# Crocodoctopus/zkstark

Hardware: AMD Instinct MI355X
Metric: field-elements/s through LDE+Merkle+FRI (full STARK-101 prover) (higher is better)
Workload: dtype u32 (mod 3*2^30+1) + SHA-256

## Files before the change

zkstark_amd/csrc/kernels.hip:

```cpp
#include "kernels.hpp"

#include <cstdlib>

#include "blake2s.hpp"
#include "field.hpp"
#include "fieldhash_f64.hpp"
#include "sha256_quad.hpp"
#include "sha256.hpp"

namespace zk {

__device__ __forceinline__ uint32_t pow_lookup(const PowTable& t, uint32_t e) {
    return mont_mul(t.hi[e >> t.lo_bits], t.lo[e & ((1u << t.lo_bits) - 1u)]);
}

constexpr uint32_t R2_MONT = R2;

__device__ uint32_t mont_inv(uint32_t a) {
    uint32_t r = R1, b = a;
    uint32_t e = P - 2;
#pragma unroll 1
    for (int i = 0; i < 32; ++i) {
        if (e & 1) r = mont_mul(r, b);
        b = mont_mul(b, b);
// ... 908 lines not shown
    }
    __syncthreads();
    for (uint32_t q = tid; q < np; q += nt) out[(size_t)q * a.out_stride] = high[q];
}
hipError_t launch_fri_final_poly_batch(const FinalPolyArgs& a, hipStream_t s, Profiler* prof) {
    if (a.log_m < 1 || a.log_m > kFinalPolyMaxLog || a.log_m > a.L || a.polys < 1 || !a.in || !a.out) return hipErrorInvalidValue;
    const uint32_t M = 1u << a.log_m;
    if (a.bound < 1 || a.bound > M || a.in_stride != M || a.out_stride != (size_t)a.bound + 1) return hipErrorInvalidValue;
    uint32_t per = (1u << kFinalPolyMaxLog) >> a.log_m;
    if (per > kFinalPolyBatchMaxPer) per = kFinalPolyBatchMaxPer;
    ScopedKernelTimer tm(prof, K_FOLD, 4.0 * (double)a.polys * (double)(M + a.bound + 1), s);
    const uint32_t most = (a.polys < per ? a.polys : per) << (a.log_m - 1);
    const uint32_t threads = most >= kFinalPolyThreads ? kFinalPolyThreads : ((most + 63u) & ~63u);
    hipLaunchKernelGGL(fri_final_poly_batch_kernel, dim3((a.polys + per - 1) / per), dim3(threads), 0, s, a, per);
    return hipGetLastError();
}


__constant__ FieldHashConsts g_fh_consts;
__constant__ FieldHashConsts64 g_fh_consts64;

template <int HASH> struct Hasher;
template <> struct Hasher<0> {
    static __device__ __forceinline__ Digest leaf(uint32_t v) { return sha256_leaf(v); }
    static __device__ __forceinline__ Digest inner(const Digest& l, const Digest& r) { return sha256_inner(l, r); }
};
template <> struct Hasher<1> {
    static __device__ __forceinline__ Digest leaf(uint32_t v) { return fieldhash_leaf64(v, g_fh_consts64); }
    static __device__ __forceinline__ Digest inner(const Digest& l, const Digest& r) { return fieldhash_inner64(l, r, g_fh_consts64); }
};
template <> struct Hasher<2> {
    static __device__ __forceinline__ Digest leaf(uint32_t v) { return blake2s_leaf(v); }
    static __device__ __forceinline__ Digest inner(const Digest& l, const Digest& r) { return blake2s_inner(l, r); }
};

struct PlainSrc {
    const uint32_t* vals;
    using Raw = uint32_t;
    __device__ __forceinline__ Raw fetch(size_t pos) const { return vals[pos]; }
    __device__ __forceinline__ uint32_t finish(const Raw& r, size_t) const { return r; }
    __device__ __forceinline__ uint32_t load(size_t pos) const { return vals[pos]; }
};
struct FoldSrc {
    FoldArgs a;
    using Raw = FoldRaw;
    __device__ __forceinline__ void prepare() { if (a.dyn) a.c_mont = *a.dyn; }
    __device__ __forceinline__ Raw fetch(size_t pos) const { return fold_fetch(a, pos); }
    __device__ __forceinline__ uint32_t finish(const Raw& r, size_t pos) const { uint32_t v = fold_finish(a, r); a.out[pos] = v; return v; }
    __device__ __forceinline__ uint32_t load(size_t pos) const { return finish(fetch(pos), pos); }
};
struct ComposeSrc {
    ComposeArgs a;
    using Raw = size_t;
    __device__ __forceinline__ Raw fetch(size_t pos) const { return pos; }
    __device__ __forceinline__ uint32_t finish(const Raw& r, size_t) const { return load(r); }
    __device__ __forceinline__ uint32_t load(size_t pos) const { uint32_t v = compose_at(a, pos); a.cp[pos] = v; return v; }
};

struct ComposeBlockSrc {
    ComposeBlockArgs b;
    using Raw = size_t;
    __device__ __forceinline__ uint32_t f_at(size_t t) const {
        const uint32_t gmask = (1u << b.lg) - 1u;
        if (t >> b.log_m) {
            const size_t v = t - ((size_t)1 << b.log_m);
            return b.halo[(v & gmask) * b.halo_stride + (v >> b.lg)];
        }
        const uint32_t log_cl = b.lg + b.log_cnt;
        const size_t piece = ((t >> log_cl) << b.lg) | (t & gmask);
        return b.a.f[(piece << b.log_cnt) | ((t & (((size_t)1 << log_cl) - 1)) >> b.lg)];
    }
    __device__ __forceinline__ Raw fetch(size_t pos) const { return pos; }
    __device__ __forceinline__ uint32_t finish(const Raw& r, size_t) const { return load(r); }
    __device__ __forceinline__ uint32_t load(size_t pos) const {
        const ComposeArgs& a = b.a;
        const size_t B = (size_t)1 << a.log_b;
        const uint32_t f0 = f_at(pos), f1 = f_at(pos + B), f2 = f_at(pos + 2 * B);
        const uint32_t x = mont_mul(pow_lookup(a.htab, b.e0 + (uint32_t)pos), a.w_mont);
        return compose_eval<false>(a, f0, f1, f2, a.inv_xm1[pos], a.inv_xm1[pos + 2 * B], x, a.zz[pos & (B - 1)], a.first, a.last, a.alpha0_mont,
                                   a.alpha1g2_mont, 0u);
    }
};

struct ComposeBatchSrc {
    ComposeArgs a;
    const BatchChal* chal;
    using Raw = size_t;
    __device__ __forceinline__ Raw fetch(size_t pos) const { return pos; }
    __device__ __forceinline__ uint32_t finish(const Raw& r, size_t) const { return load(r); }
    __device__ __forceinline__ uint32_t load(size_t pos) const {
        const size_t b = pos >> a.logN, i = pos & (((size_t)1 << a.logN) - 1);
        const BatchChal c = chal[b];
        uint32_t v = compose_core<true>(a, a.f + (b << a.logN), c.first, c.last, c.alpha0_mont, c.alpha1g2_mont, c.alpha2_mont, i);
        a.cp[pos] = v;
        return v;
    }
};
struct FoldBatchSrc {
    FoldArgs a;
    const BatchChal* chal;
    using Raw = size_t;
    __device__ __forceinline__ Raw fetch(size_t pos) const { return pos; }
    __device__ __forceinline__ uint32_t finish(const Raw& r, size_t) const { return load(r); }
    __device__ __forceinline__ uint32_t load(size_t pos) const {
        const uint32_t lh = a.log_m - 1;
        const size_t half = (size_t)1 << lh, b = pos >> lh, i = pos & (half - 1);
        const uint32_t* in = a.in + (b << a.log_m);
        uint32_t u = in[i], v = in[i + half];
        uint32_t xinv = pow_lookup(a.hinv, (uint32_t)(i << a.round));
        uint32_t s = mont_mul(add(u, v), a.inv2_mont);
        uint32_t d = mont_mul(mont_mul(sub(u, v), xinv), chal[b].c_mont);
        uint32_t r = add(s, d);
        a.out[pos] = r;
        return r;
    }
};

struct InterleaveSrc {
    const uint32_t* recv;
    uint32_t log_parts, log_cnt;
    using Raw = uint32_t;
    __device__ __forceinline__ uint32_t load(size_t pos) const {
        return recv[((pos & (((size_t)1 << log_parts) - 1)) << log_cnt) | (pos >> log_parts)];
    }
    __device__ __forceinline__ Raw fetch(size_t pos) const { return load(pos); }
    __device__ __forceinline__ uint32_t finish(const Raw& r, size_t) const { return r; }
};

template <class S> __device__ __forceinline__ auto src_prepare(S& s, int) -> decltype(s.prepare(), void()) { s.prepare(); }
template <class S> __device__ __forceinline__ void src_prepare(S&, long) {}

constexpr int kMerkleThreads = 256;
constexpr uint32_t kMerkleMaxK = 4;

__device__ __forceinline__ void store_digest(uint32_t* nodes, size_t node, const Digest& d) {
    uint4* q = reinterpret_cast<uint4*>(nodes + node * 8);
    q[0] = make_uint4(d.w[0], d.w[1], d.w[2], d.w[3]);
    q[1] = make_uint4(d.w[4], d.w[5], d.w[6], d.w[7]);
}
__device__ __forceinline__ Digest load_digest(const uint32_t* nodes, size_t node) {
    const uint4* q = reinterpret_cast<const uint4*>(nodes + node * 8);
    uint4 lo = q[0], hi = q[1];
    Digest d;
    d.w[0] = lo.x; d.w[1] = lo.y; d.w[2] = lo.z; d.w[3] = lo.w;
    d.w[4] = hi.x; d.w[5] = hi.y; d.w[6] = hi.z; d.w[7] = hi.w;
    return d;
}

__device__ __forceinline__ Digest lds_digest(const uint4* p) {
    uint4 lo = p[0], hi = p[1];
    Digest d;
    d.w[0] = lo.x; d.w[1] = lo.y; d.w[2] = lo.z; d.w[3] = lo.w;
    d.w[4] = hi.x; d.w[5] = hi.y; d.w[6] = hi.z; d.w[7] = hi.w;
    return d;
}

template <class SRC, bool LEAF, int HASH>
__global__ __launch_bounds__(kMerkleThreads) void merkle_subtree_kernel(SRC src, uint32_t* nodes,
                                                                        uint32_t depth_in, uint32_t k, size_t off) {
    extern __shared__ __attribute__((aligned(16))) uint4 stage[];
    src_prepare(src, 0);
    const uint32_t lane = threadIdx.x & 63u, wave = threadIdx.x >> 6;
    const size_t gwave = (size_t)blockIdx.x * (kMerkleThreads / 64) + wave;
    const size_t base = (gwave << (6 + k)) + off;
    const size_t in_base = ((size_t)1 << depth_in) - 1;
    uint4* my = stage + (size_t)wave * (k + 1) * 128;
    uint4* scratch = my + (size_t)k * 128;
    typename SRC::Raw raw;
    Digest dnext;
    uint32_t val = 0;
    if (LEAF) val = src.load(base + lane - off);
    else dnext = load_digest(nodes, in_base + base + lane);
#pragma unroll 1
    for (uint32_t i = 0; i < (1u << k); ++i) {
        Digest d;
        const size_t pos = base + (size_t)i * 64 + lane;
        const bool more = i + 1 < (1u << k);
        if (LEAF) {
            if (more) raw = src.fetch(pos + 64 - off);
            d = Hasher<HASH>::leaf(val);
            store_digest(nodes, in_base + pos, d);
        } else {
            d = dnext;
            if (more) dnext = load_digest(nodes, in_base + pos + 64);
        }
        uint32_t idx = i, lvl = 0;
#pragma unroll 1
        while (lvl < k) {
            uint4* left = my + lvl * 128;
            uint4* grp = (idx & 1u) ? scratch : left;
            grp[2 * lane] = make_uint4(d.w[0], d.w[1], d.w[2], d.w[3]);
            grp[2 * lane + 1] = make_uint4(d.w[4], d.w[5], d.w[6], d.w[7]);
            if (!(idx & 1u)) break;
            __builtin_amdgcn_fence(__ATOMIC_RELEASE, "wavefront");
            __builtin_amdgcn_wave_barrier();
            const uint4* x = (lane < 32u ? left : scratch - 128) + 4 * lane;
            Digest l = lds_digest(x), r = lds_digest(x + 2);
            __builtin_amdgcn_wave_barrier();
            d = Hasher<HASH>::inner(l, r);
            idx >>= 1;
            ++lvl;
            store_digest(nodes, (((size_t)1 << (depth_in - lvl)) - 1) + (base >> lvl) + (size_t)idx * 64 + lane, d);
        }
        if (LEAF && more) val = src.finish(raw, pos + 64 - off);
    }
}

template <class SRC> struct B2sSrc { static constexpr bool ok = false; };
template <> struct B2sSrc<PlainSrc> { static constexpr bool ok = true; };
template <> struct B2sSrc<ComposeSrc> { static constexpr bool ok = true; };
template <> struct B2sSrc<FoldSrc> { static constexpr bool ok = true; };

template <class SRC, bool LEAF>
__global__ __launch_bounds__(kMerkleThreads) void b2s_subtree_kernel(SRC src, uint32_t* nodes, uint32_t depth_in, uint32_t k, size_t off) {
    extern __shared__ __attribute__((aligned(16))) uint4 stage[];
    src_prepare(src, 0);
    const uint32_t lane = threadIdx.x & 63u, wave = threadIdx.x >> 6;
    const size_t gwave = (size_t)blockIdx.x * (kMerkleThreads / 64) + wave;
    const size_t base = (gwave << (6 + k)) + off;
    const size_t in_base = ((size_t)1 << depth_in) - 1;
    uint4* my = stage + (size_t)wave * (k + 1) * 128;
    uint4* scratch = my + (size_t)k * 128;
    typename SRC::Raw raw;
    Digest dnext;
    uint32_t val = 0;
    if (LEAF) val = src.load(base + lane - off);
    else dnext = load_digest(nodes, in_base + base + lane);
#pragma unroll 1
    for (uint32_t i = 0; i < (1u << k); ++i) {
        Digest d;
        const size_t pos = base + (size_t)i * 64 + lane;
        const bool more = i + 1 < (1u << k);
        if (LEAF) {
            if (more) raw = src.fetch(pos + 64 - off);
            d = blake2s_leaf(val);
            store_digest(nodes, in_base + pos, d);
        } else {
            d = dnext;
            if (more) dnext = load_digest(nodes, in_base + pos + 64);
        }
        uint32_t idx = i, lvl = 0;
#pragma unroll 1
        while (lvl < k) {
            uint4* left = my + lvl * 128;
            uint4* grp = (idx & 1u) ? scratch : left;
            grp[2 * lane] = make_uint4(d.w[0], d.w[1], d.w[2], d.w[3]);
            grp[2 * lane + 1] = make_uint4(d.w[4], d.w[5], d.w[6], d.w[7]);
            if (!(idx & 1u)) break;
            __builtin_amdgcn_fence(__ATOMIC_RELEASE, "wavefront");
            __builtin_amdgcn_wave_barrier();
            const uint4* x = (lane < 32u ? left : scratch - 128) + 4 * lane;
            const Digest l = lds_digest(x), r = lds_digest(x + 2);
            __builtin_amdgcn_wave_barrier();
            d = blake2s_inner(l, r);
            idx >>= 1;
            ++lvl;
            store_digest(nodes, (((size_t)1 << (depth_in - lvl)) - 1) + (base >> lvl) + (size_t)idx * 64 + lane, d);
        }
        if (LEAF && more) val = src.finish(raw, pos + 64 - off);
    }
}

constexpr int kWgThreads = 256;
#ifndef ZK_FIELD_ROW_MAX_NODES
#define ZK_FIELD_ROW_MAX_NODES 16
#endif
constexpr uint32_t kFieldRowMaxNodes = ZK_FIELD_ROW_MAX_NODES;
static_assert(kFieldRowMaxNodes >= 16 && kFieldRowMaxNodes <= 64, "the row form takes at most four passes of 16 nodes");
#ifndef ZK_FIELD_QUAD_MAX_NODES
#define ZK_FIELD_QUAD_MAX_NODES 64
#endif
constexpr uint32_t kFieldQuadMaxNodes = ZK_FIELD_QUAD_MAX_NODES;
static_assert(kFieldQuadMaxNodes <= 128, "the quad form takes at most two passes of 64 nodes");
#ifndef ZK_FIELD_ROW_LEAF_MAX
#define ZK_FIELD_ROW_LEAF_MAX 32
#endif
constexpr uint32_t kFieldRowLeafMax = ZK_FIELD_ROW_LEAF_MAX;
static_assert(kFieldRowLeafMax <= 64, "the row form takes at most four passes of 16 leaves");
constexpr uint32_t kWgMaxLog = 10;

__device__ __forceinline__ void lds_store(uint4* p, const Digest& d) {
    p[0] = make_uint4(d.w[0], d.w[1], d.w[2], d.w[3]);
    p[1] = make_uint4(d.w[4], d.w[5], d.w[6], d.w[7]);
}

#ifndef ZK_WG_RELAXED_PUBLISH
#define ZK_WG_RELAXED_PUBLISH 1
#endif
constexpr bool kWgRelaxedPublish = ZK_WG_RELAXED_PUBLISH != 0;
__device__ __forceinline__ void publish_node(uint32_t* nodes, size_t node, const uint4* lvl0, uint32_t tid) {
    if (tid < 8) __hip_atomic_store(nodes + node * 8 + tid, reinterpret_cast<const uint32_t*>(lvl0)[tid], __ATOMIC_RELAXED, __HIP_MEMORY_SCOPE_AGENT);
    asm volatile("s_waitcnt vmcnt(0)" ::: "memory");
}
__device__ __forceinline__ Digest load_digest_agent(const uint32_t* nodes, size_t node) {
    const unsigned long long* q = reinterpret_cast<const unsigned long long*>(nodes + node * 8);
    Digest d;
#pragma unroll
    for (int i = 0; i < 4; ++i) {
        const unsigned long long v = __hip_atomic_load(q + i, __ATOMIC_RELAXED, __HIP_MEMORY_SCOPE_AGENT);
        d.w[2 * i] = (uint32_t)v; d.w[2 * i + 1] = (uint32_t)(v >> 32);
    }
    return d;
}

#ifdef ZK_WG_TRACE
constexpr uint32_t kWgTraceSlots = 48, kWgTraceLaunches = 8192;
__device__ unsigned long long g_wg_trace[kWgTraceLaunches][kWgTraceSlots];
__device__ unsigned int g_wg_trace_n, g_wg_trace_cur;
#define WG_STAMP(slot) do { if (threadIdx.x == 0 && wg_rec < kWgTraceLaunches && (slot) < kWgTraceSlots) g_wg_trace[wg_rec][(slot)] = __builtin_amdgcn_s_memrealtime(); } while (0)
#else
#define WG_STAMP(slot) do { } while (0)
#endif

template <class SRC, bool LEAF, int HASH>
__global__ __launch_bounds__(kWgThreads) void merkle_wg_kernel(SRC src, uint32_t* nodes, uint32_t depth_in, uint32_t j,
                                                               MailArgs mail, size_t off, uint32_t j2, uint32_t lds_log) {
    extern __shared__ __attribute__((aligned(16))) uint4 lvl[];
    src_prepare(src, 0);
    uint32_t* xch = reinterpret_cast<uint32_t*>(lvl + ((size_t)2 << lds_log));
    const uint32_t tid = threadIdx.x;
    uint32_t cnt = 1u << j;
    size_t first = ((size_t)blockIdx.x << j) + off;
    uint32_t d_in = depth_in, lv = j;
    const size_t in_base = ((size_t)1 << depth_in) - 1;
    QuadLane ql;
    if (HASH == 0) ql = quad_lane(tid);
#ifdef ZK_WG_TRACE
    uint32_t wg_rec = 0xffffffffu;
    if (blockIdx.x == 0 && tid == 0) {
        wg_rec = atomicAdd(&g_wg_trace_n, 1u);
        __hip_atomic_store(&g_wg_trace_cur, wg_rec, __ATOMIC_RELAXED, __HIP_MEMORY_SCOPE_AGENT);
        if (wg_rec < kWgTraceLaunches) {
            for (uint32_t i = 0; i < kWgTraceSlots; ++i) g_wg_trace[wg_rec][i] = 0;
            g_wg_trace[wg_rec][0] = (unsigned long long)depth_in | ((unsigned long long)j << 8) | ((unsigned long long)j2 << 16) | ((unsigned long long)(LEAF ? 1 : 0) << 24) |
                                    ((unsigned long long)HASH << 25) | ((unsigned long long)(mail.mailbox ? mail.top + 1 : 0) << 26) | ((unsigned long long)gridDim.x << 32);
        }
    }
    WG_STAMP(1);
#endif
    constexpr uint32_t kPer = (1u << kWgMaxLog) / kWgThreads;
    if (LEAF && HASH == 1 && cnt <= kFieldRowLeafMax) {
        const uint32_t g = tid & 15u, grp = tid >> 4;
#pragma unroll 1
        for (uint32_t b = 0; b * 16 < cnt; ++b) {
            const uint32_t i = b * 16 + grp;
            const uint32_t ii = i < cnt ? i : 0u;
            const uint32_t v = src.finish(src.fetch(first + ii - off), first + ii - off);
            const uint32_t word = g == 0 ? v : g == 15 ? 1u : 0u;
            const uint32_t res = fieldhash_inner_row16_f64(word, g, g_fh_consts64);
            if (i < cnt && g < 8) {
                nodes[(in_base + first + i) * 8 + g] = res;
                reinterpret_cast<uint32_t*>(&lvl[2 * i])[g] = res;
            }
        }
    } else if (LEAF) {
        typename SRC::Raw raw[kPer] = {};
#pragma unroll
        for (uint32_t u = 0; u < kPer; ++u)
            if (tid + u * kWgThreads < cnt) raw[u] = src.fetch(first + tid + u * kWgThreads - off);
#pragma unroll 1
        for (uint32_t i = tid; i < cnt; i += kWgThreads) {
            const Digest d = Hasher<HASH>::leaf(src.finish(raw[0], first + i - off));
            store_digest(nodes, in_base + first + i, d);
            lds_store(&lvl[2 * i], d);
#pragma unroll
            for (uint32_t u = 0; u + 1 < kPer; ++u) raw[u] = raw[u + 1];
        }
    } else {
        Digest dd[kPer];
#pragma unroll
        for (uint32_t u = 0; u < kPer; ++u)
            if (tid + u * kWgThreads < cnt) dd[u] = load_digest(nodes, in_base + first + tid + u * kWgThreads);
#pragma unroll
        for (uint32_t u = 0; u < kPer; ++u)
            if (tid + u * kWgThreads < cnt) lds_store(&lvl[2 * (tid + u * kWgThreads)], dd[u]);
    }
    if (LEAF && mail.dump_src) __threadfence();
    __syncthreads();
    WG_STAMP(2);
#pragma unroll 1
  for (uint32_t phase = 0;; ++phase) {
#pragma unroll 1
    for (uint32_t t = 1; t <= lv; ++t) {
        const uint32_t w = cnt >> t;
        const size_t out_base = (((size_t)1 << (d_in - t)) - 1) + (first >> t);
        WG_STAMP((phase ? 24u : 2u) + t - 1u);
        if (HASH == 0 && w <= 64) {
            const uint32_t lane = tid & 63u, wave = tid >> 6;
            const uint32_t node = wave * 16 + (lane >> 4) * 4 + (lane & 3u), role = (lane >> 2) & 3u;
            const bool busy = wave * 16 < w;
            uint32_t o[4];
            if (busy) sha256_inner_quad(reinterpret_cast<const uint32_t*>(&lvl[4 * (node < w ? node : 0u)]), ql, o);
            __syncthreads();
            if (busy && node < w && role < 2) {
                const uint4 v = make_uint4(o[0], o[1], o[2], o[3]);
                lvl[2 * node + (role ^ 1u)] = v;
                reinterpret_cast<uint4*>(nodes + (out_base + node) * 8)[role ^ 1u] = v;
            }
            __syncthreads();
            continue;
        }
        if (HASH == 0 && w <= 128) {
            const bool is_main = tid < 128;
            const uint32_t node = tid & 127u;
            const bool active = node < w;
            uint32_t wv[16];
            uint32_t st[8];
            if (active) {
                Digest l = lds_digest(&lvl[4 * node]), r = lds_digest(&lvl[4 * node + 2]);
#pragma unroll
                for (int i = 0; i < 8; ++i) { wv[i] = l.w[i]; wv[8 + i] = r.w[i]; st[i] = SHA_IV[i]; }
            }
            uint32_t* xb0 = xch;
            uint32_t* xb1 = xch + 16 * 128;
            if (active) {
                if (is_main) sha256_rounds16<0>(st, wv);
                else { sha256_schedule16(wv);
#pragma unroll
                       for (int i = 0; i < 16; ++i) xb0[i * 128 + node] = wv[i]; }
            }
            __syncthreads();
            if (active) {
                if (is_main) {
#pragma unroll
                    for (int i = 0; i < 16; ++i) wv[i] = xb0[i * 128 + node];
                    sha256_rounds16<16>(st, wv);
                } else { sha256_schedule16(wv);
#pragma unroll
                         for (int i = 0; i < 16; ++i) xb1[i * 128 + node] = wv[i]; }
            }
            __syncthreads();
            if (active) {
                if (is_main) {
#pragma unroll
                    for (int i = 0; i < 16; ++i) wv[i] = xb1[i * 128 + node];
                    sha256_rounds16<32>(st, wv);
                } else { sha256_schedule16(wv);
#pragma unroll
                         for (int i = 0; i < 16; ++i) xb0[i * 128 + node] = wv[i]; }
            }
            __syncthreads();
            Digest d0;
            if (active && is_main) {
#pragma unroll
                for (int i = 0; i < 16; ++i) wv[i] = xb0[i * 128 + node];
                sha256_rounds16<48>(st, wv);
#pragma unroll
                for (int i = 0; i < 8; ++i) d0.w[i] = st[i] + SHA_IV[i];
                uint32_t pad[16] = {0x80000000u, 0, 0, 0, 0, 0, 0, 0, 0, 0, 0, 0, 0, 0, 0, 512u};
                sha256_compress(d0.w, pad);
            }
            __syncthreads();
            if (active && is_main) { lds_store(&lvl[2 * node], d0); store_digest(nodes, out_base + node, d0); }
            __syncthreads();
            continue;
        }
        if (HASH == 1 && w > kFieldRowMaxNodes && w <= kFieldQuadMaxNodes) {
            const uint32_t q = tid & 3u, grp = tid >> 2;
            uint32_t res[2][4];
#pragma unroll
            for (uint32_t b = 0; b < 2; ++b) {
                if (b * 64 >= w) break;
                const uint32_t node = b * 64 + grp;
                const uint4 v = lvl[4 * (node < w ? node : 0u) + q];
                const uint32_t in[4] = {v.x, v.y, v.z, v.w};
                fieldhash_inner_quad_f64(in, q, res[b], g_fh_consts64);
            }
            __syncthreads();
#pragma unroll
            for (uint32_t b = 0; b < 2; ++b) {
                if (b * 64 >= w) break;
                const uint32_t node = b * 64 + grp;
                if (node < w && q < 2) {
                    const uint4 o = make_uint4(res[b][0], res[b][1], res[b][2], res[b][3]);
                    lvl[2 * node + q] = o;
                    reinterpret_cast<uint4*>(nodes + (out_base + node) * 8)[q] = o;
                }
            }
            __syncthreads();
            continue;
        }
        if (HASH == 1 && w <= kFieldRowMaxNodes) {
            const uint32_t g = tid & 15u, grp = tid >> 4;
            uint32_t res[4];
#pragma unroll
            for (uint32_t b = 0; b < 4; ++b) {
                if (b * 16 >= w) break;
                const uint32_t node = b * 16 + grp;
                const uint32_t* words = reinterpret_cast<const uint32_t*>(&lvl[4 * (node < w ? node : 0u)]);
                res[b] = fieldhash_inner_row16_f64(words[g], g, g_fh_consts64);
            }
            __syncthreads();
#pragma unroll
            for (uint32_t b = 0; b < 4; ++b) {
                if (b * 16 >= w) break;
                const uint32_t node = b * 16 + grp;
                if (node < w && g < 8) {
                    reinterpret_cast<uint32_t*>(&lvl[2 * node])[g] = res[b];
                    nodes[(out_base + node) * 8 + g] = res[b];
                }
            }
            __syncthreads();
            continue;
        }
        Digest d0, d1;
        const bool a0 = tid < w, a1 = tid + kWgThreads < w;
        if (a0) d0 = Hasher<HASH>::inner(lds_digest(&lvl[4 * tid]), lds_digest(&lvl[4 * tid + 2]));
        if (a1) d1 = Hasher<HASH>::inner(lds_digest(&lvl[4 * (tid + kWgThreads)]), lds_digest(&lvl[4 * (tid + kWgThreads) + 2]));
        __syncthreads();
        if (a0) { lds_store(&lvl[2 * tid], d0); store_digest(nodes, out_base + tid, d0); }
        if (a1) { lds_store(&lvl[2 * (tid + kWgThreads)], d1); store_digest(nodes, out_base + tid + kWgThreads, d1); }
        __syncthreads();
    }
    WG_STAMP((phase ? 24u : 2u) + lv);
    if (phase == 1 || j2 == 0) break;
    __shared__ uint32_t go_on;
    if (gridDim.x > 1) {
        if (kWgRelaxedPublish) {
            publish_node(nodes, (((size_t)1 << (depth_in - j)) - 1) + blockIdx.x, lvl, tid);
        } else {
            asm volatile("s_waitcnt vmcnt(0)" ::: "memory");
            __syncthreads();
        }
    }
    if (tid == 0) {
        uint32_t last = 1;
        if (gridDim.x > 1) {
            last = (kWgRelaxedPublish ? __hip_atomic_fetch_add(mail.counter + 1, 1u, __ATOMIC_RELAXED, __HIP_MEMORY_SCOPE_AGENT)
                                      : __hip_atomic_fetch_add(mail.counter + 1, 1u, __ATOMIC_ACQ_REL, __HIP_MEMORY_SCOPE_AGENT)) == gridDim.x - 1;
            if (last) __hip_atomic_store(mail.counter + 1, 0u, __ATOMIC_RELAXED, __HIP_MEMORY_SCOPE_AGENT);
        }
        go_on = last;
    }
    __syncthreads();
    if (!go_on) return;
    if (kWgRelaxedPublish && LEAF && mail.dump_src) __builtin_amdgcn_fence(__ATOMIC_ACQUIRE, "agent");
#ifdef ZK_WG_TRACE
    if (tid == 0) wg_rec = __hip_atomic_load(&g_wg_trace_cur, __ATOMIC_RELAXED, __HIP_MEMORY_SCOPE_AGENT);
    WG_STAMP(15);
#endif
    d_in = depth_in - j; lv = j2; cnt = gridDim.x; first = 0;
    {
        const size_t base2 = ((size_t)1 << d_in) - 1;
        Digest dd[kPer];
#pragma unroll
        for (uint32_t u = 0; u < kPer; ++u)
            if (tid + u * kWgThreads < cnt)
                dd[u] = (kWgRelaxedPublish && gridDim.x > 1) ? load_digest_agent(nodes, base2 + tid + u * kWgThreads) : load_digest(nodes, base2 + tid + u * kWgThreads);
#pragma unroll
        for (uint32_t u = 0; u < kPer; ++u)
            if (tid + u * kWgThreads < cnt) lds_store(&lvl[2 * (tid + u * kWgThreads)], dd[u]);
    }
    __syncthreads();
    WG_STAMP(16);
  }
    if (mail.mailbox && depth_in - j - j2 == mail.top && off == 0) {
        __shared__ uint32_t is_last;
        const bool relaxed = kWgRelaxedPublish && gridDim.x > 1 && j2 == 0 && mail.dump_src == nullptr;
        if (relaxed) publish_node(nodes, (((size_t)1 << mail.top) - 1) + blockIdx.x, lvl, tid);
        if (tid == 0) {
            uint32_t last = 1;
            if (gridDim.x > 1 && j2 == 0) {
                last = (relaxed ? __hip_atomic_fetch_add(mail.counter, 1u, __ATOMIC_RELAXED, __HIP_MEMORY_SCOPE_AGENT)
                                : __hip_atomic_fetch_add(mail.counter, 1u, __ATOMIC_ACQ_REL, __HIP_MEMORY_SCOPE_AGENT)) == gridDim.x - 1;
                if (last) __hip_atomic_store(mail.counter, 0u, __ATOMIC_RELAXED, __HIP_MEMORY_SCOPE_AGENT);
            }
            is_last = last;
        }
        __syncthreads();
        if (is_last) {
#ifdef ZK_WG_TRACE
            if (tid == 0 && wg_rec == 0xffffffffu) wg_rec = __hip_atomic_load(&g_wg_trace_cur, __ATOMIC_RELAXED, __HIP_MEMORY_SCOPE_AGENT);
            WG_STAMP(40);
#endif
            const uint4* sq = reinterpret_cast<const uint4*>(nodes + (((size_t)1 << mail.top) - 1) * 8);
            uint4* dq = reinterpret_cast<uint4*>(mail.mailbox + kMailDigests);
            if (relaxed) {
                for (uint32_t i = tid; i < (1u << mail.top); i += kWgThreads) {
                    const Digest d = load_digest_agent(nodes, (((size_t)1 << mail.top) - 1) + i);
                    dq[2 * i] = make_uint4(d.w[0], d.w[1], d.w[2], d.w[3]);
                    dq[2 * i + 1] = make_uint4(d.w[4], d.w[5], d.w[6], d.w[7]);
                }
            } else {
                for (uint32_t i = tid; i < (2u << mail.top); i += kWgThreads) dq[i] = sq[i];
            }
            if (mail.dump_src) {
                const uint4* sv = reinterpret_cast<const uint4*>(mail.dump_src);
                uint4* dv = reinterpret_cast<uint4*>(mail.mailbox + mail.vals_off);
                for (uint32_t i = tid; i < (1u << mail.dump_log) / 4; i += kWgThreads) dv[i] = sv[i];
            }
            __threadfence_system();
            __syncthreads();
            WG_STAMP(41);
            if (tid == 0) __hip_atomic_store(&mail.mailbox[0], mail.seq, __ATOMIC_RELEASE, __HIP_MEMORY_SCOPE_SYSTEM);
            WG_STAMP(42);
        }
    }
}

#ifdef ZK_WG_TRACE
void dump_wg_trace() {
    const char* path = getenv("ZK_WG_TRACE_FILE");
    unsigned int n = 0;
    if (!path || hipMemcpyFromSymbol(&n, HIP_SYMBOL(g_wg_trace_n), sizeof n) != hipSuccess || !n) return;
    if (n > kWgTraceLaunches) n = kWgTraceLaunches;
    std::vector<unsigned long long> rec((size_t)n * kWgTraceSlots);
    if (hipMemcpyFromSymbol(rec.data(), HIP_SYMBOL(g_wg_trace), rec.size() * 8) != hipSuccess) return;
    FILE* f = fopen(path, "a");
    if (!f) return;
    for (unsigned int r = 0; r < n; ++r) {
        const unsigned long long* x = &rec[(size_t)r * kWgTraceSlots];
        const unsigned long long m = x[0];
        fprintf(f, "wg depth_in=%llu j=%llu j2=%llu leaf=%llu hash=%llu top=%lld wgs=%llu abs0=%llu :", m & 255, (m >> 8) & 255, (m >> 16) & 255, (m >> 24) & 1, (m >> 25) & 1,
                (long long)((m >> 26) & 63) - 1, m >> 32, x[1]);
        for (uint32_t i = 1; i < kWgTraceSlots; ++i) fprintf(f, " %lld", x[i] ? (long long)(x[i] - x[1]) : -1LL);
        fprintf(f, "\n");
    }
    fclose(f);
    const unsigned int zero = 0;
    (void)hipMemcpyToSymbol(HIP_SYMBOL(g_wg_trace_n), &zero, sizeof zero);
}
#endif

template <int HASH, int S>
__device__ __forceinline__ Digest coset_leaf_digest(const uint32_t (&v)[S]) {
    Digest d;
    if (HASH == ZK_HASH_BLAKE2S) {
        d = blake2s_slots<S>(v);
    } else if (HASH == ZK_HASH_FIELD) {
        uint32_t in[kFhT];
#pragma unroll
        for (int i = 0; i < kFhT; ++i) in[i] = i < S ? v[i] : 0u;
        in[kFhT - 1] = (uint32_t)S;
        fh64_compress(in, d.w, g_fh_consts64);
    } else {
        uint32_t w[16];
#pragma unroll
        for (int i = 0; i < 16; ++i) w[i] = i < S ? v[i] : 0u;
        w[S] = 0x80000000u;
        w[15] = 32u * S;
#pragma unroll
        for (int i = 0; i < 8; ++i) d.w[i] = SHA_IV[i];
        sha256_compress(d.w, w);
    }
    return d;
}
constexpr int kCosetThreads = 256;
template <int HASH, int STEPS>
__global__ __launch_bounds__(kCosetThreads) void coset_leaf_hash_kernel(const uint32_t* __restrict__ layer, uint32_t log_len, uint32_t* __restrict__ nodes) {
    constexpr int S = 1 << STEPS;
    const size_t leaves = (size_t)1 << (log_len - STEPS);
    const size_t stride = (size_t)gridDim.x * kCosetThreads;
    size_t c = (size_t)blockIdx.x * kCosetThreads + threadIdx.x;
    if (c >= leaves) return;
    uint32_t v[S], nx[S] = {};
#pragma unroll
    for (int u = 0; u < S; ++u) v[u] = layer[c + (size_t)u * leaves];
    bool more;
#pragma unroll 1
    do {
        const size_t cn = c + stride;
        more = cn < leaves;
        if (more) {
#pragma unroll
            for (int u = 0; u < S; ++u) nx[u] = layer[cn + (size_t)u * leaves];
        }
        store_digest(nodes, leaves - 1 + c, coset_leaf_digest<HASH, S>(v));
#pragma unroll
        for (int u = 0; u < S; ++u) v[u] = nx[u];
        c = cn;
    } while (more);
}

static double merkle_bytes(bool leaf, uint32_t depth, uint32_t k) {
    double in = (double)((size_t)1 << depth);
    double produced = (leaf ? in : 0.0) + in * (1.0 - 1.0 / (double)((size_t)1 << k));
    return (leaf ? 4.0 : 32.0) * in + 32.0 * produced;
}
static double hash_leaf_ops(int hash) { return hash == ZK_HASH_FIELD ? kFieldLeafOps : hash == ZK_HASH_BLAKE2S ? kB2sLeafOps : kShaLeafOps; }
static double merkle_ops(bool leaf, uint32_t depth, uint32_t k, int hash) {
    double in = (double)((size_t)1 << depth);
    double lo = hash_leaf_ops(hash), io = hash == ZK_HASH_FIELD ? kFieldInnerOps : hash == ZK_HASH_BLAKE2S ? kB2sInnerOps : kShaInnerOps;
    return (leaf ? in * lo : 0.0) + in * (1.0 - 1.0 / (double)((size_t)1 << k)) * io;
}

static hipError_t ensure_fieldhash_consts() {
    static bool done[64] = {false};
    int dev = 0;
    hipError_t e = hipGetDevice(&dev);
    if (e != hipSuccess) return e;
    if (dev < 0 || dev >= 64 || done[dev]) return hipSuccess;
    FieldHashConsts c;
    fieldhash_make_consts(c);
    e = hipMemcpyToSymbol(HIP_SYMBOL(g_fh_consts), &c, sizeof c);
    if (e != hipSuccess) return e;
    static FieldHashConsts64 c64;
    fieldhash_make_consts64(c, c64);
    e = hipMemcpyToSymbol(HIP_SYMBOL(g_fh_consts64), &c64, sizeof c64);
    if (e == hipSuccess) done[dev] = true;
    return e;
}

#ifndef ZK_MERKLE_MAX_K
#define ZK_MERKLE_MAX_K 4
#endif
#ifndef ZK_MERKLE_LATENCY_LOG
#define ZK_MERKLE_LATENCY_LOG 17
#endif
#ifndef ZK_MERKLE_CHUNK_K
#define ZK_MERKLE_CHUNK_K 3
#endif
static_assert(ZK_MERKLE_MAX_K >= 1 && ZK_MERKLE_MAX_K <= (int)kMerkleMaxK && ZK_MERKLE_CHUNK_K >= 1 && ZK_MERKLE_CHUNK_K <= (int)kMerkleMaxK, "levels per launch");
static_assert(ZK_MERKLE_LATENCY_LOG >= 12 && ZK_MERKLE_LATENCY_LOG <= 24, "latency switch");
static uint32_t g_merkle_latency_log = ZK_MERKLE_LATENCY_LOG;
static constexpr uint32_t merkle_max_k() { return ZK_MERKLE_MAX_K; }
static uint32_t merkle_latency_log() { return __atomic_load_n(&g_merkle_latency_log, __ATOMIC_RELAXED); }
bool set_merkle_latency_log(uint32_t v) {
    if (v == 0) v = ZK_MERKLE_LATENCY_LOG;
    if (v < 12 || v > 24) return false;
    __atomic_store_n(&g_merkle_latency_log, v, __ATOMIC_RELAXED);
    return true;
}

constexpr double kB2sLevelUs = kB2sInnerOps * 4.6 / kShaInnerOps, kB2sLeafUs = kB2sLeafOps * 2.6 / kShaLeafOps;
static double wg_level_us(uint32_t w, int hash) {
    if (w == 0) return 0.0;
    if (hash == ZK_HASH_BLAKE2S) return (double)((w + 255) / 256) * kB2sLevelUs;
    if (hash == ZK_HASH_FIELD) return w <= kFieldRowMaxNodes ? (double)((w + 15) / 16) * 3.7 : w <= kFieldQuadMaxNodes ? (double)((w + 63) / 64) * 5.3 : (double)((w + 255) / 256) * 10.8;
    return w <= 64 ? 3.1 : w <= 128 ? 4.9 : (double)((w + 255) / 256) * 4.6;
}
static double wg_phase_us(bool leaf, uint32_t cnt_log, uint32_t levels, int hash, uint32_t blocks) {
    const uint32_t cnt = 1u << cnt_log;
    double us = !leaf ? 1.0
                : hash == ZK_HASH_FIELD ? (cnt <= kFieldRowLeafMax ? (double)((cnt + 15) / 16) * 3.7 : (double)((cnt + 255) / 256) * 10.8)
                : (double)((cnt + 255) / 256) * (hash == ZK_HASH_BLAKE2S ? kB2sLeafUs : 2.6);
    for (uint32_t t = 1; t <= levels; ++t) us += wg_level_us(cnt >> t, hash);
    return blocks > 256 ? us * (double)blocks / 256.0 : us;
}
#ifndef ZK_MERKLE_CONTINUATION
#define ZK_MERKLE_CONTINUATION 1
#endif
static constexpr bool g_merkle_continuation = ZK_MERKLE_CONTINUATION != 0;
constexpr double kContinueUs = 6.0;
constexpr double kLaunchUs = 10.0;

template <class SRC>
static hipError_t merkle_build_t(SRC src, double src_bytes, uint32_t log_m, uint32_t* nodes, hipStream_t s, Profiler* prof,
                                 const MailArgs& mail_in, int hash, uint32_t log_sub = 0xffffffffu, size_t chunk = 0,
                                 bool leaf_mode = true, uint32_t tp_floor = 0) {
    if (hash == ZK_HASH_BLAKE2S && !B2sSrc<SRC>::ok) return hipErrorInvalidValue;
    if (hash == ZK_HASH_FIELD) {
        hipError_t e = ensure_fieldhash_consts();
        if (e != hipSuccess) return e;
    }
    if (log_sub == 0xffffffffu) log_sub = log_m;
    const uint32_t stop = log_m - log_sub;
    uint32_t depth = log_m;
    bool leaf = leaf_mode;
    const PlainSrc none{nullptr};
    auto first_bytes = [&](double b) { return leaf ? b - 4.0 * (double)((size_t)1 << log_sub) + src_bytes : b; };
    const uint32_t kMerkleLatencyLog = merkle_latency_log();
    auto off_at = [&](uint32_t d) { return (size_t)chunk << (d - stop); };
    const bool throughput_only = tp_floor != 0;
    MailArgs mail = mail_in;
    if (stop != 0 || mail.top >= log_m) mail.top = 0;
    const uint32_t end = stop == 0 ? mail.top : stop;
    const uint32_t latency_depth = stop + kMerkleLatencyLog > end ? stop + kMerkleLatencyLog : end;
    const uint32_t floor_depth = throughput_only ? tp_floor : latency_depth;
    while (depth > floor_depth) {
        uint32_t k = depth - floor_depth;
        if (k > merkle_max_k()) k = merkle_max_k();
        size_t lanes = (size_t)1 << (depth - stop - k);
        uint32_t blocks = (uint32_t)(lanes / kMerkleThreads);
        size_t sh = (size_t)(kMerkleThreads / 64) * (k + 1) * 128 * sizeof(uint4);
        ScopedKernelTimer tm(prof, leaf ? K_MERKLE_LEAF : K_MERKLE_INNER, first_bytes(merkle_bytes(leaf, depth - stop, k)), s, merkle_ops(leaf, depth - stop, k, hash));
        if (hash == ZK_HASH_BLAKE2S) {
            if constexpr (B2sSrc<SRC>::ok) {
                if (leaf) hipLaunchKernelGGL((b2s_subtree_kernel<SRC, true>), dim3(blocks), dim3(kMerkleThreads), sh, s, src, nodes, depth, k, off_at(depth));
                else hipLaunchKernelGGL((b2s_subtree_kernel<PlainSrc, false>), dim3(blocks), dim3(kMerkleThreads), sh, s, none, nodes, depth, k, off_at(depth));
            }
        } else if (hash == ZK_HASH_FIELD) {
            if (leaf) hipLaunchKernelGGL((merkle_subtree_kernel<SRC, true, 1>), dim3(blocks), dim3(kMerkleThreads), sh, s, src, nodes, depth, k, off_at(depth));
            else hipLaunchKernelGGL((merkle_subtree_kernel<PlainSrc, false, 1>), dim3(blocks), dim3(kMerkleThreads), sh, s, none, nodes, depth, k, off_at(depth));
        } else {
            if (leaf) hipLaunchKernelGGL((merkle_subtree_kernel<SRC, true, 0>), dim3(blocks), dim3(kMerkleThreads), sh, s, src, nodes, depth, k, off_at(depth));
            else hipLaunchKernelGGL((merkle_subtree_kernel<PlainSrc, false, 0>), dim3(blocks), dim3(kMerkleThreads), sh, s, none, nodes, depth, k, off_at(depth));
        }
        leaf = false;
        depth -= k;
    }
    if (throughput_only || (depth < log_m && depth <= end)) return hipGetLastError();
    auto launch_wg = [&](uint32_t j, uint32_t j2) {
        const uint32_t span = depth - stop;
        const uint32_t blocks = 1u << (span - j);
        const uint32_t lds_log = j2 && span - j > j ? span - j : j;
        const size_t sh = ((size_t)2 << lds_log) * sizeof(uint4) + 2 * 16 * 128 * sizeof(uint32_t);
        ScopedKernelTimer tm(prof, K_MERKLE_TOP, first_bytes(merkle_bytes(leaf, span, j)) + (j2 ? merkle_bytes(false, span - j, j2) : 0.0), s,
                             merkle_ops(leaf, span, j, hash) + (j2 ? merkle_ops(false, span - j, j2, hash) : 0.0));
        if (hash == ZK_HASH_BLAKE2S) {
            if constexpr (B2sSrc<SRC>::ok) {
                if (leaf) hipLaunchKernelGGL((merkle_wg_kernel<SRC, true, 2>), dim3(blocks), dim3(kWgThreads), sh, s, src, nodes, depth, j, mail, off_at(depth), j2, lds_log);
                else hipLaunchKernelGGL((merkle_wg_kernel<PlainSrc, false, 2>), dim3(blocks), dim3(kWgThreads), sh, s, none, nodes, depth, j, mail, off_at(depth), j2, lds_log);
            }
        } else if (hash == ZK_HASH_FIELD) {
            if (leaf) hipLaunchKernelGGL((merkle_wg_kernel<SRC, true, 1>), dim3(blocks), dim3(kWgThreads), sh, s, src, nodes, depth, j, mail, off_at(depth), j2, lds_log);
            else hipLaunchKernelGGL((merkle_wg_kernel<PlainSrc, false, 1>), dim3(blocks), dim3(kWgThreads), sh, s, none, nodes, depth, j, mail, off_at(depth), j2, lds_log);
        } else {
            if (leaf) hipLaunchKernelGGL((merkle_wg_kernel<SRC, true, 0>), dim3(blocks), dim3(kWgThreads), sh, s, src, nodes, depth, j, mail, off_at(depth), j2, lds_log);
            else hipLaunchKernelGGL((merkle_wg_kernel<PlainSrc, false, 0>), dim3(blocks), dim3(kWgThreads), sh, s, none, nodes, depth, j, mail, off_at(depth), j2, lds_log);
        }
        leaf = false;
        depth -= j + j2;
    };
    const bool may_continue = stop == 0 && mail.counter != nullptr && g_merkle_continuation;
    do {
        const uint32_t span = depth - stop;
        const uint32_t levels = depth - end;
        const uint32_t launches = levels ? (levels + kWgMaxLog - 1) / kWgMaxLog : 1;
        const uint32_t jn = (levels + launches - 1) / launches;
        uint32_t best_j = jn, best_j2 = 0;
        if (may_continue && levels <= 2 * kWgMaxLog) {
            double best = wg_phase_us(leaf, jn, jn, hash, 1u << (span - jn));
            if (launches == 2 && span - jn <= kWgMaxLog) best += kLaunchUs + wg_phase_us(false, span - jn, levels - jn, hash, 1);
            else if (launches > 1) best = 0.0;
            for (uint32_t j = 1; j < levels && j <= kWgMaxLog; ++j) {
                const uint32_t j2 = levels - j;
                if (j2 > kWgMaxLog || span - j > kWgMaxLog) continue;
                const double us = wg_phase_us(leaf, j, j, hash, 1u << (span - j)) + kContinueUs + wg_phase_us(false, span - j, j2, hash, 1);
                if (us < best) { best = us; best_j = j; best_j2 = j2; }
            }
        }
        launch_wg(best_j, best_j2);
    } while (depth > end);
    return hipGetLastError();
}

hipError_t launch_merkle_build(const uint32_t* vals, uint32_t log_m, uint32_t* nodes, hipStream_t s, Profiler* prof,
                               const MailArgs& mail, int hash) {
    return merkle_build_t(PlainSrc{vals}, 4.0 * (double)((size_t)1 << log_m), log_m, nodes, s, prof, mail, hash);
}
template <int HASH>
static void coset_leaf_launch(const uint32_t* vals, uint32_t log_len, uint32_t steps, uint32_t* nodes, uint32_t blocks, hipStream_t s) {
    const dim3 g(blocks), b(kCosetThreads);
    if (steps == 1) hipLaunchKernelGGL((coset_leaf_hash_kernel<HASH, 1>), g, b, 0, s, vals, log_len, nodes);
    else if (steps == 2) hipLaunchKernelGGL((coset_leaf_hash_kernel<HASH, 2>), g, b, 0, s, vals, log_len, nodes);
    else hipLaunchKernelGGL((coset_leaf_hash_kernel<HASH, 3>), g, b, 0, s, vals, log_len, nodes);
}
hipError_t launch_merkle_build_coset(const uint32_t* vals, uint32_t log_len, uint32_t steps, uint32_t* nodes, hipStream_t s, Profiler* prof,
                                     const MailArgs& mail, int hash) {
    if (steps == 0) return launch_merkle_build(vals, log_len, nodes, s, prof, mail, hash);
    if (steps > 3 || log_len <= steps) return hipErrorInvalidValue;
    if (hash == ZK_HASH_FIELD) {
        hipError_t e = ensure_fieldhash_consts();
        if (e != hipSuccess) return e;
    }
    const uint32_t log_m = log_len - steps;
    const size_t leaves = (size_t)1 << log_m;
    const size_t lanes = leaves > 4 * (size_t)kCosetThreads ? leaves / 4 : leaves;
    const uint32_t blocks = (uint32_t)((lanes + kCosetThreads - 1) / kCosetThreads);
    {
        ScopedKernelTimer tm(prof, K_MERKLE_LEAF, 4.0 * (double)((size_t)1 << log_len) + 32.0 * (double)leaves, s,
                             (double)leaves * hash_leaf_ops(hash));
        if (hash == ZK_HASH_BLAKE2S) coset_leaf_launch<2>(vals, log_len, steps, nodes, blocks, s);
        else if (hash == ZK_HASH_FIELD) coset_leaf_launch<1>(vals, log_len, steps, nodes, blocks, s);
        else coset_leaf_launch<0>(vals, log_len, steps, nodes, blocks, s);
    }
    hipError_t e = hipGetLastError();
    if (e != hipSuccess) return e;
    return merkle_build_t(PlainSrc{nullptr}, 0.0, log_m, nodes, s, prof, mail, hash, log_m, 0, false);
}
template <int HASH, int STEPS>
__global__ __launch_bounds__(kCosetThreads) void coset_leaf_hash_batch_kernel(const uint32_t* __restrict__ vals, uint32_t log_len, uint32_t log_batch,
                                                                              uint32_t* __restrict__ nodes) {
    constexpr int S = 1 << STEPS;
    const uint32_t log_m = log_len - STEPS;
    const size_t m = (size_t)1 << log_m;
    const size_t total = m << log_batch;
    const size_t stride = (size_t)gridDim.x * kCosetThreads;
    size_t g = (size_t)blockIdx.x * kCosetThreads + threadIdx.x;
    if (g >= total) return;
    uint32_t v[S], nx[S] = {};
    {
        const uint32_t* src = vals + ((g >> log_m) << log_len) + (g & (m - 1));
#pragma unroll
        for (int u = 0; u < S; ++u) v[u] = src[(size_t)u * m];
    }
    bool more;
#pragma unroll 1
    do {
        const size_t gn = g + stride;
        more = gn < total;
        if (more) {
            const uint32_t* src = vals + ((gn >> log_m) << log_len) + (gn & (m - 1));
#pragma unroll
            for (int u = 0; u < S; ++u) nx[u] = src[(size_t)u * m];
        }
        store_digest(nodes, total - 1 + g, coset_leaf_digest<HASH, S>(v));
// ... 514 lines not shown
```

Before: 2.912 billion.

## Publish leaf values with relaxed atomics and merge mailbox copy loops

Leaf values destined for the host mailbox are now written with relaxed agent-scope atomic stores during leaf hashing. This replaces the device-wide threadfence and acquire fence, and lets the relaxed publish path also run when values are dumped. The final mailbox copy now moves digests and values in one loop using buffer loads with a cache-policy flag. The old system-scope threadfence is replaced by a wave-level waitcnt plus a single release fence before a relaxed system-scope store. These changes aim to cut fence and serialization cost in the mailbox path, but rely on subtle memory-ordering reasoning that could break host visibility.

Result: no change. 2.947 billion (median of 6 runs) (+1.2%).

```diff
diff --git a/zkstark_amd/csrc/kernels.hip b/zkstark_amd/csrc/kernels.hip
--- a/zkstark_amd/csrc/kernels.hip
+++ b/zkstark_amd/csrc/kernels.hip
@@ -1234,6 +1234,18 @@
     }
     return d;
 }
+__device__ __forceinline__ uint4 load16_agent(const void* base, uint32_t bytes, uint32_t off) {
+    typedef uint32_t u32x4 __attribute__((ext_vector_type(4)));
+    const __amdgpu_buffer_rsrc_t rsrc = __builtin_amdgcn_make_buffer_rsrc(const_cast<void*>(base), 0, bytes, 0x00020000);
+    const u32x4 v = __builtin_amdgcn_raw_buffer_load_b128(rsrc, off, 0, 16);
+    return make_uint4(v.x, v.y, v.z, v.w);
+}
+__device__ __forceinline__ bool wg_values_cross(const MailArgs& mail, bool leaf) {
+    return kWgRelaxedPublish && leaf && mail.dump_src != nullptr && gridDim.x > 1;
+}
+__device__ __forceinline__ void publish_value(const MailArgs& mail, size_t pos, uint32_t v) {
+    __hip_atomic_store(const_cast<uint32_t*>(mail.dump_src) + pos, v, __ATOMIC_RELAXED, __HIP_MEMORY_SCOPE_AGENT);
+}
 
 #ifdef ZK_WG_TRACE
 constexpr uint32_t kWgTraceSlots = 48, kWgTraceLaunches = 8192;
@@ -1271,6 +1283,7 @@
     WG_STAMP(1);
 #endif
     constexpr uint32_t kPer = (1u << kWgMaxLog) / kWgThreads;
+    const bool vals_cross = wg_values_cross(mail, LEAF);
     if (LEAF && HASH == 1 && cnt <= kFieldRowLeafMax) {
         const uint32_t g = tid & 15u, grp = tid >> 4;
 #pragma unroll 1
@@ -1284,6 +1297,7 @@
                 nodes[(in_base + first + i) * 8 + g] = res;
                 reinterpret_cast<uint32_t*>(&lvl[2 * i])[g] = res;
             }
+            if (vals_cross && i < cnt && g == 0) publish_value(mail, first + i - off, v);
         }
     } else if (LEAF) {
         typename SRC::Raw raw[kPer] = {};
@@ -1292,7 +1306,9 @@
             if (tid + u * kWgThreads < cnt) raw[u] = src.fetch(first + tid + u * kWgThreads - off);
 #pragma unroll 1
         for (uint32_t i = tid; i < cnt; i += kWgThreads) {
-            const Digest d = Hasher<HASH>::leaf(src.finish(raw[0], first + i - off));
+            const uint32_t v = src.finish(raw[0], first + i - off);
+            if (vals_cross) publish_value(mail, first + i - off, v);
+            const Digest d = Hasher<HASH>::leaf(v);
             store_digest(nodes, in_base + first + i, d);
             lds_store(&lvl[2 * i], d);
 #pragma unroll
@@ -1307,7 +1323,8 @@
         for (uint32_t u = 0; u < kPer; ++u)
             if (tid + u * kWgThreads < cnt) lds_store(&lvl[2 * (tid + u * kWgThreads)], dd[u]);
     }
-    if (LEAF && mail.dump_src) __threadfence();
+    if (vals_cross) asm volatile("s_waitcnt vmcnt(0)" ::: "memory");
+    if (!kWgRelaxedPublish && LEAF && mail.dump_src) __threadfence();
     __syncthreads();
     WG_STAMP(2);
 #pragma unroll 1
@@ -1466,7 +1483,6 @@
     }
     __syncthreads();
     if (!go_on) return;
-    if (kWgRelaxedPublish && LEAF && mail.dump_src) __builtin_amdgcn_fence(__ATOMIC_ACQUIRE, "agent");
 #ifdef ZK_WG_TRACE
     if (tid == 0) wg_rec = __hip_atomic_load(&g_wg_trace_cur, __ATOMIC_RELAXED, __HIP_MEMORY_SCOPE_AGENT);
     WG_STAMP(15);
@@ -1488,7 +1504,7 @@
   }
     if (mail.mailbox && depth_in - j - j2 == mail.top && off == 0) {
         __shared__ uint32_t is_last;
-        const bool relaxed = kWgRelaxedPublish && gridDim.x > 1 && j2 == 0 && mail.dump_src == nullptr;
+        const bool relaxed = kWgRelaxedPublish && gridDim.x > 1 && j2 == 0;
         if (relaxed) publish_node(nodes, (((size_t)1 << mail.top) - 1) + blockIdx.x, lvl, tid);
         if (tid == 0) {
             uint32_t last = 1;
@@ -1506,25 +1522,28 @@
             WG_STAMP(40);
 #endif
             const uint4* sq = reinterpret_cast<const uint4*>(nodes + (((size_t)1 << mail.top) - 1) * 8);
+            const uint4* sv = reinterpret_cast<const uint4*>(mail.dump_src);
             uint4* dq = reinterpret_cast<uint4*>(mail.mailbox + kMailDigests);
-            if (relaxed) {
-                for (uint32_t i = tid; i < (1u << mail.top); i += kWgThreads) {
-                    const Digest d = load_digest_agent(nodes, (((size_t)1 << mail.top) - 1) + i);
-                    dq[2 * i] = make_uint4(d.w[0], d.w[1], d.w[2], d.w[3]);
-                    dq[2 * i + 1] = make_uint4(d.w[4], d.w[5], d.w[6], d.w[7]);
+            uint4* dv = reinterpret_cast<uint4*>(mail.mailbox + mail.vals_off);
+            const uint32_t nd = 1u << mail.top, nv = mail.dump_src ? (1u << mail.dump_log) / 4 : 0u;
+            for (uint32_t i = tid; i < nd || i < nv; i += kWgThreads) {
+                uint4 a = {}, b = {}, v = {};
+                if (i < nd) {
+                    a = relaxed ? load16_agent(sq, 32 * nd, 32 * i) : sq[2 * i];
+                    b = relaxed ? load16_agent(sq, 32 * nd, 32 * i + 16) : sq[2 * i + 1];
                 }
-            } else {
-                for (uint32_t i = tid; i < (2u << mail.top); i += kWgThreads) dq[i] = sq[i];
-            }
-            if (mail.dump_src) {
-                const uint4* sv = reinterpret_cast<const uint4*>(mail.dump_src);
-                uint4* dv = reinterpret_cast<uint4*>(mail.mailbox + mail.vals_off);
-                for (uint32_t i = tid; i < (1u << mail.dump_log) / 4; i += kWgThreads) dv[i] = sv[i];
-            }
-            __threadfence_system();
+                if (i < nv) v = vals_cross ? load16_agent(sv, 16 * nv, 16 * i) : sv[i];
+                if (i < nd) { dq[2 * i] = a; dq[2 * i + 1] = b; }
+                if (i < nv) dv[i] = v;
+            }
+            asm volatile("s_waitcnt vmcnt(0)" ::: "memory");
             __syncthreads();
             WG_STAMP(41);
-            if (tid == 0) __hip_atomic_store(&mail.mailbox[0], mail.seq, __ATOMIC_RELEASE, __HIP_MEMORY_SCOPE_SYSTEM);
+            if (tid == 0) {
+                __builtin_amdgcn_fence(__ATOMIC_RELEASE, "");
+                asm volatile("s_waitcnt vmcnt(0)" ::: "memory");
+                __hip_atomic_store(&mail.mailbox[0], mail.seq, __ATOMIC_RELAXED, __HIP_MEMORY_SCOPE_SYSTEM);
+            }
             WG_STAMP(42);
         }
     }
```
